# XiangFeng-Wen/STF-Unet

Measured on AMD Instinct MI355X. Metric: training samples/sec (256x256 DCE-MRI frames), higher is better.
Workload: dtype bf16; 1 GPU; cfg2 UNet(in=8,base_c=64) 256x256 train step; model=UNet, global_batch=64, per_gpu_batch=64, seq_len=8, parallelism=dp1, ddp_hook=False

## Files before the change

### include/stfunet.h

```cpp
#ifndef STFUNET_H
#define STFUNET_H
#include <stddef.h>
#include <stdint.h>

#ifdef __cplusplus
extern "C" {
#endif

typedef void* stf_stream_t;

typedef struct stf_conv_geom {
  int N;
  int Hs, Ws, Cs;
  int src_cstride;
  int Hd, Wd;
  int R, S;
  int stride, pad;
  int transposed;
} stf_conv_geom;

typedef struct stf_lstm_epi {
  const float* c_prev;
  float* c_out;
  void* h_out;
// ... 66 lines not shown
                    float* scale, float* shift, stf_stream_t stream);
typedef struct stf_bn_run_desc {
  const float* stats;
  float* running_mean;
  float* running_var;
  int64_t Mg;
  int tiles, groups, C;
  float momentum;
} stf_bn_run_desc;
int stf_bn_running_batch(const stf_bn_run_desc* descs, int count, stf_stream_t stream);
int stf_bn_act(const void* y, int y_cstride, int N, int H, int W, int C, int groups,
               const float* scale, const float* shift, int relu, const void* res,
               int res_cstride, const float* res_scale, const float* res_shift, void* out,
               int out_cstride, void* pooled, stf_stream_t stream);
int stf_bn_bwd_tiles(int N, int H, int W, int C, int groups, int pooled);
int stf_bn_bwd_reduce(const void* dz, int dz_cstride, const void* dpool, const void* y,
                      int y_cstride, int N, int H, int W, int C, int groups,
                      const float* scale, const float* shift, const float* mean,
                      const float* invstd, int mask_mode, const void* mask_src,
                      int mask_cstride, void* g_out, float* partial, stf_stream_t stream);
int stf_bn_bwd_finalize(float* partial, int tiles, int groups, int C, int64_t M,
                        const float* gamma, const float* mean, const float* invstd,
                        float* dgamma, float* dbeta, float* coef, stf_stream_t stream);
typedef struct stf_bn_gsum_desc {
  const float* partial;
  float* dgamma;
  float* dbeta;
  int tiles, groups, C;
} stf_bn_gsum_desc;
int stf_bn_groupsum_batch(const stf_bn_gsum_desc* descs, int count, stf_stream_t stream);
int stf_bn_bwd_apply_tiles(int64_t M, int C);
int stf_bn_bwd_apply(const void* g, int g_cstride, const void* y, int y_cstride, int64_t M,
                     int C, int groups, const float* mask_scale, const float* mask_shift,
                     const float* coef, void* dy, int dy_cstride, float* bias_partial,
                     float* dbias, stf_stream_t stream);

int stf_head_fwd(const void* y, int N, int H, int W, int C, const float* scale,
                 const float* shift, const float* w, const float* bias, int classes,
                 float* logits, stf_stream_t stream);
int stf_head_bwd(const float* dlogits, const void* y, int N, int H, int W, int C,
                 const float* scale, const float* shift, const float* mean,
                 const float* invstd, const float* w, int classes, void* g_out,
                 float* bn_partial, float* head_partial, float* dw, float* db,
                 stf_stream_t stream);
int stf_head_tiles(int N, int H, int W, int C);

// ... 276 lines not shown
```

### stf-unet_amd/csrc/bn.hip

```cpp
#include <algorithm>

#include "common.h"
#include "../../include/stfunet.h"
#include "reduce.h"

namespace {

constexpr int NT = 256;

STF_DEV void bn_fin_store(int g, int c, int C, double mu, double var, const float* gamma, const float* beta,
                          float eps, float* mean, float* invstd, float* scale, float* shift) {
  const float inv = (float)(1.0 / sqrt(var + (double)eps));
  const float sc = gamma[c] * inv;
  mean[g * C + c] = (float)mu;
  invstd[g * C + c] = inv;
  scale[g * C + c] = sc;
  shift[g * C + c] = beta[c] - (float)mu * sc;
}

STF_DEV void bn_fin_fwd_out(float* base, int g, int c, int G, int C, long Mg, double s1, double s2,
                            const float* gamma, const float* beta, float mom, float eps, float* rm, float* rv,
                            float* mean, float* invstd, float* scale, float* shift) {
  const double mu = s1 / Mg;
  double var = s2 / Mg - mu * mu;
// ... 29 lines not shown
  if (!lead) return;
  bn_fin_store(g, c, C, rm ? rm[c] : 0.f, rv ? rv[c] : 1.f, gamma, beta, eps, mean, invstd, scale, shift);
}

STF_DEV void bn_fin_bwd_out(float* base, int g, int c, int G, int C, long Mg, double s1, double s2,
                            const float* gamma, const float* mean, const float* invstd, float* dgamma, float* dbeta,
                            float* coef) {
  const double is = invstd[g * C + c];
  const double A = (double)gamma[c] * is;
  const double B = -A * is * s2 / Mg;
  const double Cc = -A * s1 / Mg + A * is * mean[g * C + c] * s2 / Mg;
  coef[(size_t)g * 3 * C + c] = (float)A;
  coef[(size_t)g * 3 * C + C + c] = (float)B;
  coef[(size_t)g * 3 * C + 2 * C + c] = (float)Cc;
  if (G == 1) {
    if (dgamma) dgamma[c] = (float)s2;
    if (dbeta) dbeta[c] = (float)s1;
  } else {
    base[c] = (float)s1;
    base[C + c] = (float)s2;
  }
}


STF_DEV void load_pair(const float* a, const float* b, int g, int C, int cg, float (&va)[8], float (&vb)[8]) {
  load8f(a + (size_t)g * C, cg * 8, va);
  load8f(b + (size_t)g * C, cg * 8, vb);
}
STF_DEV void load_coef(const float* coef, int g, int C, int cg, float (&A)[8], float (&B)[8], float (&Cc)[8]) {
  load8f(coef + (size_t)g * 3 * C, cg * 8, A);
  load8f(coef + (size_t)g * 3 * C + C, cg * 8, B);
  load8f(coef + (size_t)g * 3 * C + 2 * C, cg * 8, Cc);
}

STF_DEV void bn_affine8(float (&v)[8], const float (&sc)[8], const float (&sh)[8], int relu, int res_mode,
                        const uint4* rq, const float (&rs)[8], const float (&rh)[8]) {
#pragma unroll
  for (int j = 0; j < 8; ++j) v[j] = v[j] * sc[j] + sh[j];
  if (res_mode) {
    float r[8];
    unpack8(*rq, r);
    if (res_mode == 2) {
#pragma unroll
      for (int j = 0; j < 8; ++j) r[j] = r[j] * rs[j] + rh[j];
    }
#pragma unroll
// ... 11 lines not shown
  for (int j = 0; j < 8; ++j) {
    bool keep = true;
    if (mask == 1) keep = y[j] * sc[j] + sh[j] > 0.f;
    else if (mask == 2) keep = mk[j] > 0.f;
    const float gj = keep ? d[j] : 0.f;
    d[j] = gj;
    sg[j] += gj;
    sgx[j] += gj * (y[j] - mu[j]) * is[j];
  }
}

STF_DEV void bn_dy8(bool mask, float (&gv)[8], const float (&y)[8], const float (&ms)[8], const float (&mh)[8],
                    const float (&A)[8], const float (&B)[8], const float (&Cc)[8], float (&sb)[8]) {
#pragma unroll
  for (int j = 0; j < 8; ++j) {
    const float gj = (mask && !(y[j] * ms[j] + mh[j] > 0.f)) ? 0.f : gv[j];
    gv[j] = A[j] * gj + B[j] * y[j] + Cc[j];
    sb[j] += gv[j];
  }
}

template <int Q = 1, int NTH, int RW>
STF_DEV void bn_block_fold(float (&red)[NTH][RW], const float (&s0)[8], const float (&s1)[8], int C, int stride,
                           int gy, float* __restrict__ out) {
  constexpr int H = (RW - 1) / 8;
#pragma unroll
  for (int j = 0; j < 8; ++j) {
    red[threadIdx.x][j] = s0[j];
    if (H == 2) red[threadIdx.x][8 + j] = s1[j];
  }
  __syncthreads();
  const size_t row = (size_t)gy * gridDim.x + blockIdx.x;
  for (int c = threadIdx.x; c < C; c += NTH) {
    const int gg = c >> 3, j = c & 7;
    float a = 0.f, b = 0.f;
    for (int t = Q * gg; t < NTH; t += stride)
      for (int q = 0; q < Q; ++q) {
        a += red[t + q][j];
        if (H == 2) b += red[t + q][8 + j];
      }
    out[row * H * C + c] = a;
    if (H == 2) out[row * H * C + C + c] = b;
  }
}

template <bool POOL>
__global__ void bn_act_kernel(const uint16_t* __restrict__ y, int ycs, long N, int H, int W, int C, long Mg,
                              const float* scale, const float* shift, int relu, int res_mode,
                              const uint16_t* __restrict__ res, int rcs, const float* __restrict__ rscale,
                              const float* __restrict__ rshift, uint16_t* __restrict__ out, int ocs,
                              uint16_t* __restrict__ pooled) {
  const int CG = C / 8;
  const long units = POOL ? N * (H / 2) * (W / 2) * CG : N * H * W * CG;
  for (long u = blockIdx.x * (long)NT + threadIdx.x; u < units; u += (long)gridDim.x * NT) {
    const int cg = (int)(u % CG);
    const long pix = u / CG;
    if (!POOL) {
      const int g = (int)(pix / Mg);
      float sc[8], sh[8], v[8];
      load_pair(scale, shift, g, C, cg, sc, sh);
      unpack8(*reinterpret_cast<const uint4*>(y + pix * ycs + cg * 8), v);
#pragma unroll
      for (int j = 0; j < 8; ++j) v[j] = v[j] * sc[j] + sh[j];
      if (res_mode) {
        float r[8];
// ... 102 lines not shown
        sg[j] += t;
        sgx[j] += t * (v[d][j] - mu[j]) * is[j];
      }
      *reinterpret_cast<uint4*>(g_out + p[d] * C + cg * 8) = pack8(gd);
    }
  }
  bn_block_fold(red, sg, sgx, C, CG, 0, partial);
}

STF_DEV float quad_xor1(float v) {
  return __int_as_float(__builtin_amdgcn_mov_dpp(__float_as_int(v), 0xB1, 0xF, 0xF, false));
}
STF_DEV float quad_xor2(float v) {
  return __int_as_float(__builtin_amdgcn_mov_dpp(__float_as_int(v), 0x4E, 0xF, 0xF, false));
}

constexpr int PNT = 512;
__global__ __launch_bounds__(PNT) void bn_bwd_reduce_pool_kernel(const uint16_t* __restrict__ dz, int dzcs,
                                          const uint16_t* __restrict__ dpool, const uint16_t* __restrict__ y,
                                          int ycs, long N, int H, int W, int C, int G, int tpg,
                                          const float* __restrict__ scale, const float* __restrict__ shift,
                                          const float* __restrict__ mean, const float* __restrict__ invstd,
                                          int mask_mode, uint16_t* __restrict__ g_out,
                                          float* __restrict__ partial) {
  __shared__ float red[PNT][17];
  const int CG = C / 8;
  const int g = blockIdx.x / tpg, tile = blockIdx.x - g * tpg;
  const int Wp = W / 2, Hp = H / 2;
  const long wpg = (N / G) * Hp * Wp;
  const long U = wpg * CG * 4;
  const long gt = (long)tile * PNT + threadIdx.x;
  const int d = (int)(gt & 3);
  const int cg = (int)((gt >> 2) % CG);
  float sc[8], sh[8], mu[8], is[8];
  load_pair(scale, shift, g, C, cg, sc, sh);
  load_pair(mean, invstd, g, C, cg, mu, is);
  const bool relu = mask_mode == 1;
  float sg[8] = {0, 0, 0, 0, 0, 0, 0, 0}, sgx[8] = {0, 0, 0, 0, 0, 0, 0, 0};
  const int HpWp = Hp * Wp, cshift = __builtin_ctz(CG);
  const long S = (long)tpg * PNT;
  auto pix = [&](long u, int& win) {
    win = (int)(u >> (2 + cshift)) + (int)(g * wpg);
    const int n = win / HpWp;
    const int rem = win - n * HpWp;
    const int py = rem / Wp, px = rem - py * Wp;
    return ((long)(n * H + 2 * py + (d >> 1))) * W + 2 * px + (d & 1);
  };
  auto unit = [&](long p, int win, const uint4& yv, const uint4& zv, const uint4& pv) {
// ... 20 lines not shown
      sg[j] += gj;
      sgx[j] += gj * (v[j] - mu[j]) * is[j];
    }
    *reinterpret_cast<uint4*>(g_out + p * C + cg * 8) = pack8(gd);
  };
  const uint4 zero4 = make_uint4(0, 0, 0, 0);
  for (long u = gt; u < U; u += 2 * S) {
    const bool two = u + S < U;
    int w0, w1 = 0;
    const long p0 = pix(u, w0);
    const long p1 = two ? pix(u + S, w1) : p0;
    const uint4 y0 = *reinterpret_cast<const uint4*>(y + p0 * ycs + cg * 8);
    const uint4 z0 = dz ? *reinterpret_cast<const uint4*>(dz + p0 * dzcs + cg * 8) : zero4;
    const uint4 q0 = *reinterpret_cast<const uint4*>(dpool + (long)w0 * C + cg * 8);
    uint4 y1 = zero4, z1 = zero4, q1 = zero4;
    if (two) {
      y1 = *reinterpret_cast<const uint4*>(y + p1 * ycs + cg * 8);
      if (dz) z1 = *reinterpret_cast<const uint4*>(dz + p1 * dzcs + cg * 8);
      q1 = *reinterpret_cast<const uint4*>(dpool + (long)w1 * C + cg * 8);
    }
    unit(p0, w0, y0, z0, q0);
    if (two) unit(p1, w1, y1, z1, q1);
  }
  bn_block_fold<4>(red, sg, sgx, C, 4 * CG, 0, partial);
}

__global__ __launch_bounds__(stf::FOLD_NT) void bn_bwd_finalize_kernel(float* __restrict__ partial, int S, int T, int G,
                                                            int C, long Mg, const float* gamma, const float* mean,
                                                            const float* invstd, float* dgamma, float* dbeta,
                                                            float* coef) {
  __shared__ double red[stf::FOLD_NT];
  const int g = blockIdx.y;
  const int c = blockIdx.x * 16 + (threadIdx.x & 15);
  const bool cok = c < C, lead = cok && (threadIdx.x >> 4) == 0;
  float* base = partial + (size_t)g * T * 2 * C;
  double s1, s2;
  stf::fold16_pair(base, S, 2L * C, C, c, cok, red, s1, s2);
  if (lead) bn_fin_bwd_out(base, g, c, G, C, Mg, s1, s2, gamma, mean, invstd, dgamma, dbeta, coef);
}

constexpr int RUN_BATCH = 32;
struct RunBatch { stf_bn_run_desc d[RUN_BATCH]; };
__global__ void bn_running_batch_kernel(RunBatch b) {
  const stf_bn_run_desc& d = b.d[blockIdx.y];
  const int c = blockIdx.x * blockDim.x + threadIdx.x;
  if (c >= d.C) return;
  float run_m = d.running_mean[c], run_v = d.running_var[c];
// ... 52 lines not shown
        if (RES) rv[k] = *reinterpret_cast<const uint4*>(res + p * rcs + cg * 8);
      }
    }
#pragma unroll
    for (int k = 0; k < UPT; ++k) {
      const int uk = u + k * NT;
      if (uk >= upg) break;
      float v[8];
      unpack8(yv[k], v);
      bn_affine8(v, sc, sh, relu, RES ? (res_mode == 2 ? 2 : 1) : 0, &rv[k], rs, rh);
      *reinterpret_cast<uint4*>(out + (p0 + (uk >> cgs)) * ocs + cg * 8) = pack8(v);
    }
  }
}

template <int MASK>
__global__ __launch_bounds__(NT) void bn_bwd_reduce_g_kernel(const uint16_t* __restrict__ dz, int dzcs,
                                                             const uint16_t* __restrict__ y, int ycs, int Mg,
                                                             int cgs, const float* __restrict__ scale,
                                                             const float* __restrict__ shift,
                                                             const float* __restrict__ mean,
                                                             const float* __restrict__ invstd,
                                                             const uint16_t* __restrict__ msrc, int mcs,
                                                             uint16_t* __restrict__ g_out, float* __restrict__ partial) {
  __shared__ float red[NT][17];
  const int g = blockIdx.y, CG = 1 << cgs, C = 8 << cgs;
  const int upg = Mg << cgs, S = gridDim.x * NT * UPT;
  const int u0 = blockIdx.x * NT * UPT + threadIdx.x;
  const int cg = threadIdx.x & (CG - 1);
  float sc[8], sh[8], mu[8], is[8];
  if (MASK == 1) load_pair(scale, shift, g, C, cg, sc, sh);
  load_pair(mean, invstd, g, C, cg, mu, is);
  float sg[8] = {0, 0, 0, 0, 0, 0, 0, 0}, sgx[8] = {0, 0, 0, 0, 0, 0, 0, 0};
  const size_t p0 = (size_t)g * Mg;
  for (int u = u0; u < upg; u += S) {
    uint4 yv[UPT], zv[UPT], mv[UPT];
#pragma unroll
    for (int k = 0; k < UPT; ++k) {
      const int uk = u + k * NT;
      if (uk < upg) {
        const size_t p = p0 + (uk >> cgs);
        yv[k] = *reinterpret_cast<const uint4*>(y + p * ycs + cg * 8);
        zv[k] = *reinterpret_cast<const uint4*>(dz + p * dzcs + cg * 8);
        if (MASK == 2) mv[k] = *reinterpret_cast<const uint4*>(msrc + p * mcs + cg * 8);
      }
    }
#pragma unroll
    for (int k = 0; k < UPT; ++k) {
      const int uk = u + k * NT;
      if (uk >= upg) break;
      float v[8], d[8], mk[8];
      unpack8(yv[k], v);
      unpack8(zv[k], d);
      if (MASK == 2) unpack8(mv[k], mk);
      bn_acc8(MASK, d, v, sc, sh, mk, mu, is, sg, sgx);
      if (g_out) *reinterpret_cast<uint4*>(g_out + (p0 + (uk >> cgs)) * C + cg * 8) = pack8(d);
    }
  }
  bn_block_fold(red, sg, sgx, C, CG, g, partial);
}

template <bool MASK>
__global__ __launch_bounds__(NT) void bn_bwd_apply_g_kernel(const uint16_t* g_in, int gcs,
                                                            const uint16_t* __restrict__ y, int ycs, int Mg, int cgs,
                                                            const float* coef, const float* __restrict__ mscale,
                                                            const float* __restrict__ mshift, uint16_t* dy,
                                                            int dycs, float* __restrict__ bias_partial) {
  __shared__ float red[NT][9];
  const int g = blockIdx.y, CG = 1 << cgs, C = 8 << cgs;
  const int upg = Mg << cgs, S = gridDim.x * NT * UPT;
  const int u0 = blockIdx.x * NT * UPT + threadIdx.x;
  const int cg = threadIdx.x & (CG - 1);
  float A[8], B[8], Cc[8], ms[8], mh[8];
  load_coef(coef, g, C, cg, A, B, Cc);
  if (MASK) load_pair(mscale, mshift, g, C, cg, ms, mh);
  float sb[8] = {0, 0, 0, 0, 0, 0, 0, 0};
  const size_t p0 = (size_t)g * Mg;
  for (int u = u0; u < upg; u += S) {
    uint4 gq[UPT], yq[UPT];
#pragma unroll
    for (int k = 0; k < UPT; ++k) {
      const int uk = u + k * NT;
// ... 161 lines not shown
enum class BnOp { Act, Reduce, Apply, ActPool3, ReducePool3, ApplyPool3 };
struct BnSig {
  BnOp op;
  long N;
  int H, W, C, groups;
  bool pooled = false;
  int mask = 0;
  bool res = false;
  bool bias = false;
};
enum class BnKernel {
  None, ActG, ActGRes, ActFlat, ActFlatPool, ReduceG0, ReduceG1, ReduceG2, ReduceDpp, ReduceWin, ApplyG, ApplyGMask,
  ActPool3, ReducePool3, ApplyPool3
};
struct BnRoute {
  bool refused = true;
  BnKernel kernel = BnKernel::None;
  int block = NT;
  dim3 grid;
  int rows = 0;
  int alloc = 1;
  int cgs = 0;
  long Mg = 0;
};

constexpr long ROW_CAP = stf::FOLD16_ROWS, BLOCK_CAP = 8192, IDX_CAP = 1L << 31;

BnRoute bn_route(const BnSig& s) {
  BnRoute r;
  if (s.groups < 1) return r;
  const auto clamp = [](long want, long most) { return (int)std::max<long>(1, std::min(want, most)); };
  const auto ceil_div = [](long x, long y) { return (x + y - 1) / y; };
  const int CG = s.C / 8, Ho = (s.H - 1) / 2 + 1, Wo = (s.W - 1) / 2 + 1;
  const long Ng = s.N / s.groups, px = s.N * s.H * s.W;
  r.Mg = Ng * s.H * s.W;
  const bool chunk_ok = s.C >= 8 && s.C % 8 == 0 && NT % CG == 0;
  const bool g_ok = chunk_ok && r.Mg * CG < IDX_CAP;
  if (chunk_ok) r.cgs = 31 - __builtin_clz(CG);
  const bool uneven = s.N % s.groups != 0, odd = ((s.H | s.W) & 1) != 0;
  const long upg = Ng * CG * (s.op == BnOp::ApplyPool3 ? (long)((s.H + 1) / 2) * ((s.W + 1) / 2)
                              : s.pooled ? (long)(s.H / 2) * (s.W / 2) : (long)s.H * s.W);
  const auto rows_of = [&](long units) { return clamp(ceil_div(units, NT), ceil_div(ROW_CAP, s.groups)); };
  const auto blocks_of = [&](long cap) { return clamp(ceil_div(upg, (long)NT * UPT), cap / s.groups); };
  const auto flat = [&](long units) { return (unsigned)std::min(ceil_div(units, NT), BLOCK_CAP); };
  switch (s.op) {
    case BnOp::Act:
      r.refused = s.C % 8 || uneven || (s.pooled && (odd || s.res));
      if (!s.pooled && g_ok) {
        r.kernel = s.res ? BnKernel::ActGRes : BnKernel::ActG;
        r.grid = dim3(upg ? blocks_of(BLOCK_CAP) : 0, s.groups);
      } else {
        r.kernel = s.pooled ? BnKernel::ActFlatPool : BnKernel::ActFlat;
        r.grid = dim3(flat(upg * s.groups));
      }
      break;
    case BnOp::Reduce:
      r.refused = !chunk_ok || uneven || (s.pooled ? odd || s.mask == 2 : !g_ok);
      r.rows = r.alloc = rows_of(upg);
      if (!s.pooled) {
        r.kernel = s.mask == 1 ? BnKernel::ReduceG1 : s.mask == 2 ? BnKernel::ReduceG2 : BnKernel::ReduceG0;
        r.grid = dim3(r.rows, s.groups);
      } else {
        const bool dpp = chunk_ok && 64 % CG == 0 && px < IDX_CAP;
        r.kernel = dpp ? BnKernel::ReduceDpp : BnKernel::ReduceWin;
        r.block = dpp ? PNT : NT;
        r.grid = dim3(r.rows * s.groups);
      }
      break;
    case BnOp::Apply:
      r.alloc = clamp(ceil_div(px * CG, NT), ROW_CAP);
      r.rows = blocks_of(s.bias ? r.alloc : BLOCK_CAP);
      r.refused = !g_ok || uneven || (s.bias && (long)r.rows * s.groups > r.alloc);
      r.kernel = s.mask ? BnKernel::ApplyGMask : BnKernel::ApplyG;
      r.grid = dim3(r.rows, s.groups);
      if (!s.bias) r.rows = 0;
      break;
    case BnOp::ActPool3: {
      const long units = s.N * Ho * Wo * CG;
      r.refused = s.C % 8 || uneven || units >= IDX_CAP - BLOCK_CAP * NT || px * s.C >= IDX_CAP * 8;
      r.kernel = BnKernel::ActPool3;
      r.grid = dim3(std::max(flat(units), 1u));
      break;
    }
    case BnOp::ReducePool3:
      r.refused = !g_ok || uneven || px >= IDX_CAP;
      r.kernel = BnKernel::ReducePool3;
      r.rows = r.alloc = rows_of(r.Mg * CG);
      r.grid = dim3(r.rows, s.groups);
      break;
    case BnOp::ApplyPool3:
// ... 49 lines not shown
                       r.cgs, scale, shift, relu, res_mode, (const uint16_t*)res, res_cstride, res_scale, res_shift,
                       (uint16_t*)out, out_cstride);
  };
  const auto flat = [&](auto kernel) {
    hipLaunchKernelGGL(kernel, r.grid, dim3(r.block), 0, (hipStream_t)stream, (const uint16_t*)y, y_cstride, (long)N, H,
                       W, C, r.Mg, scale, shift, relu, res_mode, (const uint16_t*)res, res_cstride, res_scale,
                       res_shift, (uint16_t*)out, out_cstride, (uint16_t*)pooled);
  };
  switch (r.kernel) {
    case BnKernel::ActG: group_major(bn_act_g_kernel<false>); break;
    case BnKernel::ActGRes: group_major(bn_act_g_kernel<true>); break;
    case BnKernel::ActFlat: flat(bn_act_kernel<false>); break;
    case BnKernel::ActFlatPool: flat(bn_act_kernel<true>); break;
    default: return STF_EINVAL;
  }
  STF_CHECK_LAUNCH();
  return 0;
}

extern "C" int stf_bn_bwd_tiles(int N, int H, int W, int C, int groups, int pooled) {
  return bn_route({BnOp::Reduce, N, H, W, C, groups, pooled != 0}).alloc;
}

extern "C" int stf_bn_bwd_reduce(const void* dz, int dz_cstride, const void* dpool, const void* y, int y_cstride,
                                 int N, int H, int W, int C, int groups, const float* scale, const float* shift,
                                 const float* mean, const float* invstd, int mask_mode, const void* mask_src,
                                 int mask_cstride, void* g_out, float* partial, stf_stream_t stream) {
  const BnRoute r = bn_route({BnOp::Reduce, N, H, W, C, groups, dpool != nullptr, mask_mode});
  if (r.refused || y_cstride % 8 || (dz && dz_cstride % 8)) return STF_EINVAL;
  if (!dz && !dpool) return STF_EINVAL;
  if (!g_out && dpool) return STF_EINVAL;
  if (mask_mode == 2 && (!mask_src || mask_cstride % 8)) return STF_EINVAL;
  hipStream_t s = (hipStream_t)stream;
  const auto group_major = [&](auto kernel) {
    hipLaunchKernelGGL(kernel, r.grid, dim3(r.block), 0, s, (const uint16_t*)dz, dz_cstride, (const uint16_t*)y,
                       y_cstride, (int)r.Mg, r.cgs, scale, shift, mean, invstd, (const uint16_t*)mask_src,
                       mask_cstride, (uint16_t*)g_out, partial);
  };
  switch (r.kernel) {
    case BnKernel::ReduceG0: group_major(bn_bwd_reduce_g_kernel<0>); break;
    case BnKernel::ReduceG1: group_major(bn_bwd_reduce_g_kernel<1>); break;
    case BnKernel::ReduceG2: group_major(bn_bwd_reduce_g_kernel<2>); break;
    case BnKernel::ReduceDpp:
      hipLaunchKernelGGL(bn_bwd_reduce_pool_kernel, r.grid, dim3(r.block), 0, s, (const uint16_t*)dz, dz_cstride,
                         (const uint16_t*)dpool, (const uint16_t*)y, y_cstride, (long)N, H, W, C, groups, r.rows, scale,
                         shift, mean, invstd, mask_mode, (uint16_t*)g_out, partial);
      break;
    case BnKernel::ReduceWin:
      hipLaunchKernelGGL(bn_bwd_reduce_win_kernel, r.grid, dim3(r.block), 0, s, (const uint16_t*)dz, dz_cstride,
                         (const uint16_t*)dpool, (const uint16_t*)y, y_cstride, (long)N, H, W, C, groups, r.rows, scale,
                         shift, mean, invstd, mask_mode, (const uint16_t*)mask_src, mask_cstride, (uint16_t*)g_out,
                         partial);
      break;
    default: return STF_EINVAL;
  }
  STF_CHECK_LAUNCH();
  return 0;
}

extern "C" int stf_bn_bwd_finalize(float* partial, int tiles, int groups, int C, int64_t M, const float* gamma,
                                   const float* mean, const float* invstd, float* dgamma, float* dbeta, float* coef,
                                   stf_stream_t stream) {
  hipStream_t s = (hipStream_t)stream;
  if (groups < 1 || M % groups) return STF_EINVAL;
  const int S = stf::colsum_stage1(partial, tiles, 2L * C, s, groups, stf::FOLD16_ROWS);
  hipLaunchKernelGGL(bn_bwd_finalize_kernel, dim3((C + 15) / 16, groups), dim3(stf::FOLD_NT), 0, s, partial, S, tiles, groups,
                     C, (long)(M / groups), gamma, mean, invstd, dgamma, dbeta, coef);
  STF_CHECK_LAUNCH();
  if (groups > 1 && (dgamma || dbeta)) {
    GsumBatch b;
    b.d[0] = stf_bn_gsum_desc{partial, dgamma, dbeta, tiles, groups, C};
    hipLaunchKernelGGL(bn_groupsum_batch_kernel, dim3((C + 255) / 256, 1), dim3(256), 0, s, b);
    STF_CHECK_LAUNCH();
  }
  return 0;
}

extern "C" int stf_bn_running_batch(const stf_bn_run_desc* descs, int count, stf_stream_t stream) {
  for (int i = 0; i < count; ++i)
    if (!descs[i].stats || !descs[i].running_mean || !descs[i].running_var || descs[i].groups < 1 ||
// ... 96 lines not shown
```

### stf-unet_amd/csrc/reduce.h

```cpp
#pragma once
#include "common.h"

namespace stf {

static __global__ void colsum_inplace_kernel(float* __restrict__ buf, long T, long W, int S) {
  const long j = blockIdx.x * (long)blockDim.x + threadIdx.x;
  const int s = blockIdx.y;
  if (j >= W) return;
  float* b = buf + (size_t)blockIdx.z * T * W;
  double acc = 0.0;
  for (long t = s; t < T; t += S) acc += b[t * W + j];
  b[(long)s * W + j] = (float)acc;
}

static inline int colsum_split(long T, long W, int G) {
  long s = T / 64;
  const long blocks_x = (W + 255) / 256;
  if (blocks_x * s * G < 512) s = T / 16;
  if (s < 1) s = 1;
  if (s > 256) s = 256;
  if (s > T) s = (int)T;
  return (int)s;
}

// ... 12 lines not shown
    int t = threadIdx.x >> 4;
    for (; t + 3 * RL < S; t += 4 * RL) {
      a0 += base[(long)t * stride + c];
      a1 += base[(long)(t + RL) * stride + c];
      a2 += base[(long)(t + 2 * RL) * stride + c];
      a3 += base[(long)(t + 3 * RL) * stride + c];
    }
    for (; t < S; t += RL) a0 += base[(long)t * stride + c];
  }
  return (a0 + a1) + (a2 + a3);
}

STF_DEV double fold16_finish(double v, double* red) {
  red[threadIdx.x] = v;
  __syncthreads();
  double tot = 0.0;
  const int RL = blockDim.x >> 4;
  if ((threadIdx.x >> 4) == 0)
    for (int r = 0; r < RL; ++r) tot += red[r * 16 + (threadIdx.x & 15)];
  __syncthreads();
  return tot;
}

STF_DEV void fold16_pair(const float* base, int S, long stride, long off2, long c, bool cok, double* red,
                         double& o1, double& o2) {
  double a0 = 0.0, a1 = 0.0, b0 = 0.0, b1 = 0.0;
  if (cok) {
    const int RL = blockDim.x >> 4;
    int t = threadIdx.x >> 4;
    for (; t + RL < S; t += 2 * RL) {
      const float x0 = base[(long)t * stride + c], y0 = base[(long)t * stride + off2 + c];
      const float x1 = base[(long)(t + RL) * stride + c], y1 = base[(long)(t + RL) * stride + off2 + c];
      a0 += x0; b0 += y0; a1 += x1; b1 += y1;
    }
    for (; t < S; t += RL) {
      a0 += base[(long)t * stride + c];
      b0 += base[(long)t * stride + off2 + c];
    }
  }
  double v1 = a0 + a1, v2 = b0 + b1;
  v1 += __shfl_xor(v1, 16, 64);
  v2 += __shfl_xor(v2, 16, 64);
  v1 += __shfl_xor(v1, 32, 64);
  v2 += __shfl_xor(v2, 32, 64);
  const int wave = threadIdx.x >> 6, nw = blockDim.x >> 6, lane = threadIdx.x & 63;
  if (lane < 16) {
    red[wave * 16 + lane] = v1;
    red[(nw + wave) * 16 + lane] = v2;
  }
  __syncthreads();
  o1 = o2 = 0.0;
  if (threadIdx.x < 16)
    for (int w = 0; w < nw; ++w) {
      o1 += red[w * 16 + threadIdx.x];
      o2 += red[(nw + w) * 16 + threadIdx.x];
    }
}

constexpr int FOLD_NT = 1024;

constexpr long FOLD16_ROWS = 1024;

}
```

### stf-unet_amd/stfunet/_lib.py

```python
import contextlib
import ctypes
import os

import torch

_HERE = os.path.dirname(os.path.abspath(__file__))
LIB_PATH = os.path.join(_HERE, "libstfunet_hip.so")
LIB_PATH = os.environ.get("STF_LIB", LIB_PATH)
LIB_PATH_F16 = os.environ.get("STF_LIB_F16", os.path.join(os.path.dirname(LIB_PATH), "libstfunet_hip_f16.so"))
LIB_PATHS = {torch.bfloat16: LIB_PATH, torch.float16: LIB_PATH_F16}
STORAGE_CODE = {torch.bfloat16: 0, torch.float16: 1}

BUILD_INFO = os.path.join(_HERE, "build_info.json")
_SRC_DIRS = (os.path.join(_HERE, "..", "csrc"), os.path.join(_HERE, "..", "..", "include"))


def _sha(paths):
    import hashlib
    h = hashlib.sha256()
    for p in paths:
        h.update(os.path.basename(p).encode())
        with open(p, "rb") as f:
            h.update(f.read())
    return h.hexdigest()[:16]
# ... 68 lines not shown
    _fields_ = [("model", P), ("off", c_int64), ("len", c_int64)]


_SIGS = {
    "stf_igemm_stat_tiles": (c_int, [ctypes.POINTER(IgemmArgs)]),
    "stf_igemm_ws_bytes": (c_size_t, [ctypes.POINTER(IgemmArgs)]),
    "stf_igemm_bnr_tiles": (c_int, [ctypes.POINTER(IgemmArgs)]),
    "stf_igemm_kernel_name": (ctypes.c_char_p, [ctypes.POINTER(IgemmArgs)]),
    "stf_wgrad_kernel_name": (ctypes.c_char_p, [ctypes.POINTER(WgradArgs)]),
    "stf_igemm": (c_int, [ctypes.POINTER(IgemmArgs), P]),
    "stf_wgrad_plan": (c_int, [ctypes.POINTER(WgradArgs), ctypes.POINTER(c_int), ctypes.POINTER(c_size_t)]),
    "stf_wgrad": (c_int, [ctypes.POINTER(WgradArgs), P]),
    "stf_wgrad_reduce": (c_int, [P, c_int, c_int, c_int, c_int, c_int, P, P]),
    "stf_channel_sum": (c_int, [P, c_int, c_int, c_int, P, P, P]),
    "stf_bn_finalize": (c_int, [P, c_int, c_int, c_int, c_int64, P, P, c_float, c_float, P, P, P, P, P, P, P]),
    "stf_bn_running_batch": (c_int, [P, c_int, P]),
    "stf_bn_groupsum_batch": (c_int, [P, c_int, P]),
    "stf_bn_act": (c_int, [P, c_int, c_int, c_int, c_int, c_int, c_int, P, P, c_int, P, c_int, P, P, P, c_int, P,
                           P]),
    "stf_bn_bwd_tiles": (c_int, [c_int, c_int, c_int, c_int, c_int, c_int]),
    "stf_bn_bwd_reduce": (c_int, [P, c_int, P, P, c_int, c_int, c_int, c_int, c_int, c_int, P, P, P, P, c_int, P,
                                  c_int, P, P, P]),
    "stf_bn_bwd_finalize": (c_int, [P, c_int, c_int, c_int, c_int64, P, P, P, P, P, P, P]),
    "stf_bn_bwd_apply_tiles": (c_int, [c_int64, c_int]),
    "stf_bn_bwd_apply": (c_int, [P, c_int, P, c_int, c_int64, c_int, c_int, P, P, P, P, c_int, P, P, P]),
    "stf_head_fwd": (c_int, [P, c_int, c_int, c_int, c_int, P, P, P, P, c_int, P, P]),
    "stf_head_bwd": (c_int, [P, P, c_int, c_int, c_int, c_int, P, P, P, P, P, c_int, P, P, P, P, P, P]),
    "stf_head_tiles": (c_int, [c_int, c_int, c_int, c_int]),
    "stf_loss_scratch_floats": (c_int, [c_int, c_int]),
    "stf_loss_fwd": (c_int, [P, P, c_int, c_int, c_int, c_int, P, P, P]),
    "stf_loss_bwd": (c_int, [P, P, c_int, c_int, c_int, c_int, P, P, P, P]),
    "stf_loss_opt_scratch_floats": (c_int, [c_int, c_int]),
    "stf_loss_opt_fwd": (c_int, [P, P, c_int, c_int, c_int, c_int, P, c_int, c_int, P, P, P]),
    "stf_loss_opt_bwd": (c_int, [P, P, c_int, c_int, c_int, c_int, P, c_int, c_int, P, P, P, P]),
    "stf_head_mc_fwd": (c_int, [P, c_int, c_int, c_int, c_int, P, P, P, P, c_int, P, P]),
    "stf_head_mc_bwd": (c_int, [P, P, c_int, c_int, c_int, c_int, P, P, P, P, P, c_int, P, P, P, P, P, P]),
    "stf_loss_mc_scratch_floats": (c_int, [c_int, c_int]),
    "stf_loss_mc_fwd": (c_int, [P, P, c_int, c_int, c_int, c_int, P, c_int, c_int, P, P, P]),
    "stf_loss_mc_bwd": (c_int, [P, P, c_int, c_int, c_int, c_int, P, c_int, c_int, P, P, P, P]),
    "stf_loss_ft_scratch_floats": (c_int, [c_int, c_int]),
    "stf_loss_ft_fwd": (c_int, [P, P, c_int, c_int, c_int, c_int, P, c_int, c_int, c_float, c_float, c_float, P, P,
                                P]),
    "stf_loss_ft_bwd": (c_int, [P, P, c_int, c_int, c_int, c_int, P, c_int, c_int, c_float, c_float, c_float, P, P,
                                P, P]),
    "stf_adamw": (c_int, [P, P, P, P, c_int64, c_float, c_float, c_float, c_float, c_float, c_float, c_float,
                          P]),
# ... 195 lines not shown
```

### stf-unet_amd/stfunet/nhwc.py

```python
import contextlib
import ctypes
import os
from dataclasses import dataclass

import torch

from . import _lib
from ._lib import BnrEpi, ConvGeom, IgemmArgs, WgradArgs, call, stream

BF16 = torch.bfloat16


def sdt():
    return _lib.storage_dtype()


def _p(t):
    return t.data_ptr() if t is not None else None


class KernelTimer:

    def __init__(self, only=None, log=False):
        self.rec = {}
# ... 555 lines not shown
         _p(res_st.scale) if res_st is not None else None, _p(res_st.shift) if res_st is not None else None,
         out.ptr(), out.cs, pooled.ptr() if pooled is not None else None, stream())


def bn_backward(y: Feat, st: BNState, bn, dgamma, dbeta, dz: Feat = None, dpool: Feat = None, relu=True,
                dbias=None, mask: Feat = None, out: Feat = None, keep_g=False):
    y.check()
    C = y.C
    dev = y.buf.device
    G = st.groups
    tiles = _lib.load().stf_bn_bwd_tiles(y.N, y.H, y.W, C, G, int(dpool is not None))
    part = empty(G * tiles * 2 * C, torch.float32, dev)
    if dz is not None:
        dz.check()
        assert (dz.N, dz.H, dz.W, dz.C) == (y.N, y.H, y.W, C)
    if dpool is not None:
        dpool.check()
        assert dpool.cs == C and dpool.off == 0 and (dpool.H, dpool.W) == (y.H // 2, y.W // 2)
    mode = 2 if mask is not None else (1 if relu else 0)
    if mask is not None:
        mask.check()
    direct = dpool is None and mode != 2 and not keep_g
    g = None if direct else new_feat(y.N, y.H, y.W, C, dev)
    call("stf_bn_bwd_reduce", dz.ptr() if dz is not None else None, dz.cs if dz is not None else 0,
         dpool.ptr() if dpool is not None else None, y.ptr(), y.cs, y.N, y.H, y.W, C, G, _p(st.scale),
         _p(st.shift), _p(st.mean), _p(st.invstd), mode, mask.ptr() if mask is not None else None,
         mask.cs if mask is not None else 0, g.ptr() if g is not None else None, _p(part), stream())
    if keep_g and out is None:
        out = new_feat(y.N, y.H, y.W, C, dev)
    if direct:
        if out is None:
            out = new_feat(y.N, y.H, y.W, C, dev)
        dy = bn_backward_from_partial(dz, y, st, bn, part, tiles, dgamma, dbeta, dbias, out=out,
                                      mask_relu=(mode == 1))
    else:
        dy = bn_backward_from_partial(g, y, st, bn, part, tiles, dgamma, dbeta, dbias, out=out)
    return (dy, g) if keep_g else dy


def bn_backward_fused(dz: Feat, y: Feat, st: BNState, bn, part, tiles, dgamma, dbeta, dbias=None, relu=True):
    assert dz.cs == dz.C and dz.off == 0
    return bn_backward_from_partial(dz, y, st, bn, part, tiles, dgamma, dbeta, dbias, out=dz if relu else None,
                                    mask_relu=relu)


def bn_backward_maxpool3(y: Feat, st: BNState, bn, dgamma, dbeta, argmax, dpool: Feat):
    y.check()
    dpool.check()
    C, dev, G = y.C, y.buf.device, st.groups
    assert y.cs == C and y.off == 0 and dpool.cs == C and dpool.off == 0
    assert (dpool.N, dpool.H, dpool.W) == (y.N, (y.H - 1) // 2 + 1, (y.W - 1) // 2 + 1)
    tiles = _lib.load().stf_bn_bwd_tiles(y.N, y.H, y.W, C, G, 0)
    part = empty(G * tiles * 2 * C, torch.float32, dev)
    call("stf_bn_bwd_reduce_pool3", _p(argmax), dpool.ptr(), y.ptr(), y.N, y.H, y.W, C, G, _p(st.scale),
         _p(st.shift), _p(st.mean), _p(st.invstd), _p(part), stream())
    coef = _bn_bwd_coef(y, st, bn, part, tiles, dgamma, dbeta)
    dy = new_feat(y.N, y.H, y.W, C, dev)
    call("stf_bn_bwd_apply_pool3", _p(argmax), dpool.ptr(), y.ptr(), y.N, y.H, y.W, C, G, _p(st.scale),
         _p(st.shift), _p(coef), dy.ptr(), stream())
    return dy


def _bn_bwd_coef(y: Feat, st: BNState, bn, part, tiles, dgamma, dbeta):
    C, dev, G = y.C, y.buf.device, st.groups
    coef = empty(G * 3 * C, torch.float32, dev)
    if G > 1 and (dgamma is not None or dbeta is not None):
        _GSUM_PENDING.append((_GsumDesc(part.data_ptr(), dgamma.data_ptr() if dgamma is not None else None,
                                        dbeta.data_ptr() if dbeta is not None else None, tiles, G, C), part))
        dgamma = dbeta = None
    call("stf_bn_bwd_finalize", _p(part), tiles, G, C, y.M, bn.weight.data_ptr(), _p(st.mean),
         _p(st.invstd), _p(dgamma), _p(dbeta), _p(coef), stream())
    if not st.training:
        cv = coef.view(G, 3, C)
        cv[:, 0].copy_(bn.weight.detach() * st.invstd)
        cv[:, 1:].zero_()
    return coef


def bn_backward_from_partial(g: Feat, y: Feat, st: BNState, bn, part, tiles, dgamma, dbeta, dbias=None,
                             out: Feat = None, mask_relu=False):
    C = y.C
    dev = y.buf.device
    G = st.groups
    if st.training:
        dbias = None
    coef = _bn_bwd_coef(y, st, bn, part, tiles, dgamma, dbeta)
    bpart = None
    if dbias is not None:
        bpart = empty(_lib.load().stf_bn_bwd_apply_tiles(y.M, C) * C, torch.float32, dev)
    dst = out if out is not None else g
    if out is not None:
        out.check()
        assert (out.N, out.H, out.W, out.C) == (y.N, y.H, y.W, C)
    if mask_relu:
        assert out is not None
    call("stf_bn_bwd_apply", g.ptr(), g.cs, y.ptr(), y.cs, y.M, C, G, _p(st.scale) if mask_relu else None,
         _p(st.shift) if mask_relu else None, _p(coef), dst.ptr(), dst.cs, _p(bpart), _p(dbias), stream())
    return dst


MAX_CLASSES = 16


def check_num_classes(K):
    if not 1 <= K <= MAX_CLASSES:
        raise ValueError(f"num_classes={K}: the head and criterion kernels take 1 to {MAX_CLASSES} classes")


def _head_entry(name, K):
# ... 26 lines not shown
```

Before: 2728 samples/s.

## Fuse BN backward finalize into reduce kernel via last-block atomic fold

BN backward reduce kernels now publish their per-block partials with agent-scope atomic stores and count arrivals on a per-stream device counter. The last block to arrive folds all partials and writes dgamma, dbeta and the backward coefficients, so the separate finalize launch is skipped for single-group training layers with enough blocks. This removes one kernel launch and its dependency gap per BN layer in backward. In exchange it adds a global atomic, a fence, and a serial tail fold inside one block, which needs correct memory ordering.

```diff
diff --git a/include/stfunet.h b/include/stfunet.h
--- a/include/stfunet.h
+++ b/include/stfunet.h
@@ -112,6 +112,13 @@
 int stf_bn_bwd_finalize(float* partial, int tiles, int groups, int C, int64_t M,
                         const float* gamma, const float* mean, const float* invstd,
                         float* dgamma, float* dbeta, float* coef, stf_stream_t stream);
+int stf_bn_bwd_fold(int N, int H, int W, int C, int groups, int pooled, int training);
+int stf_bn_bwd_reduce_fin(const void* dz, int dz_cstride, const void* dpool, const void* y,
+                          int y_cstride, int N, int H, int W, int C, const float* scale,
+                          const float* shift, const float* mean, const float* invstd,
+                          int mask_mode, const void* mask_src, int mask_cstride, void* g_out,
+                          float* partial, const float* gamma, float* dgamma, float* dbeta,
+                          float* coef, stf_stream_t stream);
 typedef struct stf_bn_gsum_desc {
   const float* partial;
   float* dgamma;
diff --git a/stf-unet_amd/csrc/bn.hip b/stf-unet_amd/csrc/bn.hip
--- a/stf-unet_amd/csrc/bn.hip
+++ b/stf-unet_amd/csrc/bn.hip
@@ -75,6 +75,29 @@
   }
 }
 
+struct BwdFin {
+  const float* gamma;
+  float *dgamma, *dbeta, *coef;
+  unsigned* counter;
+  long Mg;
+};
+
+template <int NTH>
+STF_DEV void bn_bwd_fin_last(float* lds, float* partial, int rows, int C, const BwdFin& f, const float* mean,
+                             const float* invstd) {
+  static_assert(2 * (stf::FOLD_NT / 64) * 16 * sizeof(double) < (NTH * 17 - 1) * sizeof(float), "fold scratch");
+  if (!stf::arrive_last(f.counter, gridDim.x * gridDim.y, reinterpret_cast<unsigned*>(lds) + NTH * 17 - 1)) return;
+  double* red = reinterpret_cast<double*>(lds);
+  for (int c0 = 0; c0 < C; c0 += 16) {
+    const int c = c0 + (threadIdx.x & 15);
+    const bool cok = c < C;
+    double s1, s2;
+    stf::fold16_pair_as<NTH>(partial, rows, 2L * C, C, c, cok, red, s1, s2);
+    if (cok && threadIdx.x < 16)
+      bn_fin_bwd_out(partial, 0, c, 1, C, f.Mg, s1, s2, f.gamma, mean, invstd, f.dgamma, f.dbeta, f.coef);
+  }
+}
+
 
 STF_DEV void load_pair(const float* a, const float* b, int g, int C, int cg, float (&va)[8], float (&vb)[8]) {
   load8f(a + (size_t)g * C, cg * 8, va);
@@ -132,7 +155,7 @@
 
 template <int Q = 1, int NTH, int RW>
 STF_DEV void bn_block_fold(float (&red)[NTH][RW], const float (&s0)[8], const float (&s1)[8], int C, int stride,
-                           int gy, float* __restrict__ out) {
+                           int gy, float* __restrict__ out, bool through = false) {
   constexpr int H = (RW - 1) / 8;
 #pragma unroll
   for (int j = 0; j < 8; ++j) {
@@ -149,8 +172,13 @@
         a += red[t + q][j];
         if (H == 2) b += red[t + q][8 + j];
       }
-    out[row * H * C + c] = a;
-    if (H == 2) out[row * H * C + C + c] = b;
+    if (through) {
+      __hip_atomic_store(out + row * H * C + c, a, __ATOMIC_RELAXED, __HIP_MEMORY_SCOPE_AGENT);
+      if (H == 2) __hip_atomic_store(out + row * H * C + C + c, b, __ATOMIC_RELAXED, __HIP_MEMORY_SCOPE_AGENT);
+    } else {
+      out[row * H * C + c] = a;
+      if (H == 2) out[row * H * C + C + c] = b;
+    }
   }
 }
 
@@ -299,8 +327,8 @@
                                           const float* __restrict__ scale, const float* __restrict__ shift,
                                           const float* __restrict__ mean, const float* __restrict__ invstd,
                                           int mask_mode, uint16_t* __restrict__ g_out,
-                                          float* __restrict__ partial) {
-  __shared__ float red[PNT][17];
+                                          float* __restrict__ partial, BwdFin fin) {
+  __shared__ __attribute__((aligned(16))) float red[PNT][17];
   const int CG = C / 8;
   const int g = blockIdx.x / tpg, tile = blockIdx.x - g * tpg;
   const int Wp = W / 2, Hp = H / 2;
@@ -367,7 +395,8 @@
     unit(p0, w0, y0, z0, q0);
     if (two) unit(p1, w1, y1, z1, q1);
   }
-  bn_block_fold<4>(red, sg, sgx, C, 4 * CG, 0, partial);
+  bn_block_fold<4>(red, sg, sgx, C, 4 * CG, 0, partial, fin.coef != nullptr);
+  if (fin.coef) bn_bwd_fin_last<PNT>(&red[0][0], partial, gridDim.x, C, fin, mean, invstd);
 }
 
 __global__ __launch_bounds__(stf::FOLD_NT) void bn_bwd_finalize_kernel(float* __restrict__ partial, int S, int T, int G,
@@ -466,8 +495,9 @@
                                                              const float* __restrict__ mean,
                                                              const float* __restrict__ invstd,
                                                              const uint16_t* __restrict__ msrc, int mcs,
-                                                             uint16_t* __restrict__ g_out, float* __restrict__ partial) {
-  __shared__ float red[NT][17];
+                                                             uint16_t* __restrict__ g_out, float* __restrict__ partial,
+                                                             BwdFin fin) {
+  __shared__ __attribute__((aligned(16))) float red[NT][17];
   const int g = blockIdx.y, CG = 1 << cgs, C = 8 << cgs;
   const int upg = Mg << cgs, S = gridDim.x * NT * UPT;
   const int u0 = blockIdx.x * NT * UPT + threadIdx.x;
@@ -501,7 +531,8 @@
       if (g_out) *reinterpret_cast<uint4*>(g_out + (p0 + (uk >> cgs)) * C + cg * 8) = pack8(d);
     }
   }
-  bn_block_fold(red, sg, sgx, C, CG, g, partial);
+  bn_block_fold(red, sg, sgx, C, CG, g, partial, fin.coef != nullptr);
+  if (fin.coef) bn_bwd_fin_last<NT>(&red[0][0], partial, gridDim.x, C, fin, mean, invstd);
 }
 
 template <bool MASK>
@@ -709,9 +740,11 @@
   int alloc = 1;
   int cgs = 0;
   long Mg = 0;
+  bool fin_ok = false;
+  bool fold = false;
 };
 
-constexpr long ROW_CAP = stf::FOLD16_ROWS, BLOCK_CAP = 8192, IDX_CAP = 1L << 31;
+constexpr long ROW_CAP = stf::FOLD16_ROWS, BLOCK_CAP = 8192, IDX_CAP = 1L << 31, FOLD_MIN_BLOCKS = 256;
 
 BnRoute bn_route(const BnSig& s) {
   BnRoute r;
@@ -753,6 +786,8 @@
         r.block = dpp ? PNT : NT;
         r.grid = dim3(r.rows * s.groups);
       }
+      r.fin_ok = !r.refused && s.groups == 1 && r.kernel != BnKernel::ReduceWin;
+      r.fold = r.fin_ok && r.rows >= FOLD_MIN_BLOCKS;
       break;
     case BnOp::Apply:
       r.alloc = clamp(ceil_div(px * CG, NT), ROW_CAP);
@@ -848,20 +883,28 @@
   return bn_route({BnOp::Reduce, N, H, W, C, groups, pooled != 0}).alloc;
 }
 
-extern "C" int stf_bn_bwd_reduce(const void* dz, int dz_cstride, const void* dpool, const void* y, int y_cstride,
-                                 int N, int H, int W, int C, int groups, const float* scale, const float* shift,
-                                 const float* mean, const float* invstd, int mask_mode, const void* mask_src,
-                                 int mask_cstride, void* g_out, float* partial, stf_stream_t stream) {
+extern "C" int stf_bn_bwd_fold(int N, int H, int W, int C, int groups, int pooled, int training) {
+  return training && bn_route({BnOp::Reduce, N, H, W, C, groups, pooled != 0}).fold;
+}
+
+static int bn_bwd_reduce(const void* dz, int dz_cstride, const void* dpool, const void* y, int y_cstride, int N,
+                         int H, int W, int C, int groups, const float* scale, const float* shift, const float* mean,
+                         const float* invstd, int mask_mode, const void* mask_src, int mask_cstride, void* g_out,
+                         float* partial, const float* gamma, float* dgamma, float* dbeta, float* coef,
+                         stf_stream_t stream) {
   const BnRoute r = bn_route({BnOp::Reduce, N, H, W, C, groups, dpool != nullptr, mask_mode});
   if (r.refused || y_cstride % 8 || (dz && dz_cstride % 8)) return STF_EINVAL;
   if (!dz && !dpool) return STF_EINVAL;
   if (!g_out && dpool) return STF_EINVAL;
   if (mask_mode == 2 && (!mask_src || mask_cstride % 8)) return STF_EINVAL;
+  if (coef && (groups != 1 || !gamma)) return STF_EINVAL;
   hipStream_t s = (hipStream_t)stream;
+  BwdFin fin{gamma, dgamma, dbeta, nullptr, nullptr, r.Mg};
+  if (coef && r.fin_ok && (fin.counter = stf::fold_counter(s)) != nullptr) fin.coef = coef;
   const auto group_major = [&](auto kernel) {
     hipLaunchKernelGGL(kernel, r.grid, dim3(r.block), 0, s, (const uint16_t*)dz, dz_cstride, (const uint16_t*)y,
                        y_cstride, (int)r.Mg, r.cgs, scale, shift, mean, invstd, (const uint16_t*)mask_src,
-                       mask_cstride, (uint16_t*)g_out, partial);
+                       mask_cstride, (uint16_t*)g_out, partial, fin);
   };
   switch (r.kernel) {
     case BnKernel::ReduceG0: group_major(bn_bwd_reduce_g_kernel<0>); break;
@@ -870,7 +913,7 @@
     case BnKernel::ReduceDpp:
       hipLaunchKernelGGL(bn_bwd_reduce_pool_kernel, r.grid, dim3(r.block), 0, s, (const uint16_t*)dz, dz_cstride,
                          (const uint16_t*)dpool, (const uint16_t*)y, y_cstride, (long)N, H, W, C, groups, r.rows, scale,
-                         shift, mean, invstd, mask_mode, (uint16_t*)g_out, partial);
+                         shift, mean, invstd, mask_mode, (uint16_t*)g_out, partial, fin);
       break;
     case BnKernel::ReduceWin:
       hipLaunchKernelGGL(bn_bwd_reduce_win_kernel, r.grid, dim3(r.block), 0, s, (const uint16_t*)dz, dz_cstride,
@@ -881,7 +924,27 @@
     default: return STF_EINVAL;
   }
   STF_CHECK_LAUNCH();
+  if (coef && !fin.coef)
+    return stf_bn_bwd_finalize(partial, r.rows, 1, C, (int64_t)r.Mg, gamma, mean, invstd, dgamma, dbeta, coef, stream);
   return 0;
+}
+
+extern "C" int stf_bn_bwd_reduce(const void* dz, int dz_cstride, const void* dpool, const void* y, int y_cstride,
+                                 int N, int H, int W, int C, int groups, const float* scale, const float* shift,
+                                 const float* mean, const float* invstd, int mask_mode, const void* mask_src,
+                                 int mask_cstride, void* g_out, float* partial, stf_stream_t stream) {
+  return bn_bwd_reduce(dz, dz_cstride, dpool, y, y_cstride, N, H, W, C, groups, scale, shift, mean, invstd, mask_mode,
+                       mask_src, mask_cstride, g_out, partial, nullptr, nullptr, nullptr, nullptr, stream);
+}
+
+extern "C" int stf_bn_bwd_reduce_fin(const void* dz, int dz_cstride, const void* dpool, const void* y, int y_cstride,
+                                     int N, int H, int W, int C, const float* scale, const float* shift,
+                                     const float* mean, const float* invstd, int mask_mode, const void* mask_src,
+                                     int mask_cstride, void* g_out, float* partial, const float* gamma,
+                                     float* dgamma, float* dbeta, float* coef, stf_stream_t stream) {
+  if (!coef) return STF_EINVAL;
+  return bn_bwd_reduce(dz, dz_cstride, dpool, y, y_cstride, N, H, W, C, 1, scale, shift, mean, invstd, mask_mode,
+                       mask_src, mask_cstride, g_out, partial, gamma, dgamma, dbeta, coef, stream);
 }
 
 extern "C" int stf_bn_bwd_finalize(float* partial, int tiles, int groups, int C, int64_t M, const float* gamma,
diff --git a/stf-unet_amd/csrc/reduce.h b/stf-unet_amd/csrc/reduce.h
--- a/stf-unet_amd/csrc/reduce.h
+++ b/stf-unet_amd/csrc/reduce.h
@@ -1,4 +1,6 @@
 #pragma once
+#include <mutex>
+
 #include "common.h"
 
 namespace stf {
@@ -58,12 +60,12 @@
   return tot;
 }
 
-STF_DEV void fold16_pair(const float* base, int S, long stride, long off2, long c, bool cok, double* red,
-                         double& o1, double& o2) {
+STF_DEV void fold16_pair_lane(const float* base, int S, long stride, long off2, long c, bool cok, double* red,
+                              int vt, int nt) {
   double a0 = 0.0, a1 = 0.0, b0 = 0.0, b1 = 0.0;
   if (cok) {
-    const int RL = blockDim.x >> 4;
-    int t = threadIdx.x >> 4;
+    const int RL = nt >> 4;
+    int t = vt >> 4;
     for (; t + RL < S; t += 2 * RL) {
       const float x0 = base[(long)t * stride + c], y0 = base[(long)t * stride + off2 + c];
       const float x1 = base[(long)(t + RL) * stride + c], y1 = base[(long)(t + RL) * stride + off2 + c];
@@ -79,12 +81,15 @@
   v2 += __shfl_xor(v2, 16, 64);
   v1 += __shfl_xor(v1, 32, 64);
   v2 += __shfl_xor(v2, 32, 64);
-  const int wave = threadIdx.x >> 6, nw = blockDim.x >> 6, lane = threadIdx.x & 63;
+  const int wave = vt >> 6, nw = nt >> 6, lane = vt & 63;
   if (lane < 16) {
     red[wave * 16 + lane] = v1;
     red[(nw + wave) * 16 + lane] = v2;
   }
-  __syncthreads();
+}
+
+STF_DEV void fold16_pair_sum(const double* red, int nt, double& o1, double& o2) {
+  const int nw = nt >> 6;
   o1 = o2 = 0.0;
   if (threadIdx.x < 16)
     for (int w = 0; w < nw; ++w) {
@@ -93,8 +98,67 @@
     }
 }
 
+STF_DEV void fold16_pair(const float* base, int S, long stride, long off2, long c, bool cok, double* red,
+                         double& o1, double& o2) {
+  fold16_pair_lane(base, S, stride, off2, c, cok, red, threadIdx.x, blockDim.x);
+  __syncthreads();
+  fold16_pair_sum(red, blockDim.x, o1, o2);
+}
+
 constexpr int FOLD_NT = 1024;
 
 constexpr long FOLD16_ROWS = 1024;
 
+template <int NTH>
+STF_DEV void fold16_pair_as(const float* base, int S, long stride, long off2, long c, bool cok, double* red,
+                            double& o1, double& o2) {
+  static_assert(NTH % 64 == 0 && FOLD_NT % NTH == 0, "whole waves, whole passes");
+  for (int vt = threadIdx.x; vt < FOLD_NT; vt += NTH) fold16_pair_lane(base, S, stride, off2, c, cok, red, vt, FOLD_NT);
+  __syncthreads();
+  fold16_pair_sum(red, FOLD_NT, o1, o2);
+  __syncthreads();
 }
+
+STF_DEV bool arrive_last(unsigned* counter, unsigned count, unsigned* flag) {
+  asm volatile("s_waitcnt vmcnt(0)" ::: "memory");
+  __syncthreads();
+  if (threadIdx.x == 0) {
+    const unsigned ticket = __hip_atomic_fetch_add(counter, 1u, __ATOMIC_RELAXED, __HIP_MEMORY_SCOPE_AGENT);
+    const bool last = ticket + 1 == count;
+    if (last) {
+      __hip_atomic_store(counter, 0u, __ATOMIC_RELAXED, __HIP_MEMORY_SCOPE_AGENT);
+      __builtin_amdgcn_fence(__ATOMIC_ACQUIRE, "agent");
+      asm volatile("s_waitcnt vmcnt(0)" ::: "memory");
+    }
+    *flag = last;
+  }
+  __syncthreads();
+  const bool last = *flag != 0;
+  __syncthreads();
+  return last;
+}
+
+constexpr int FOLD_SLOTS = 64;
+static __device__ unsigned fold_counters[FOLD_SLOTS];
+
+static inline unsigned* fold_counter(hipStream_t s) {
+  struct Key { int dev; hipStream_t s; };
+  static std::mutex mu;
+  static Key keys[FOLD_SLOTS];
+  static unsigned* base[FOLD_SLOTS];
+  static int used = 0;
+  int dev = 0;
+  if (hipGetDevice(&dev) != hipSuccess) return nullptr;
+  std::lock_guard<std::mutex> lock(mu);
+  for (int i = 0; i < used; ++i)
+    if (keys[i].dev == dev && keys[i].s == s) return base[i] + i;
+  if (used == FOLD_SLOTS) return nullptr;
+  void* p = nullptr;
+  if (hipGetSymbolAddress(&p, HIP_SYMBOL(fold_counters)) != hipSuccess || !p) return nullptr;
+  const int i = used++;
+  keys[i] = Key{dev, s};
+  base[i] = (unsigned*)p;
+  return base[i] + i;
+}
+
+}
diff --git a/stf-unet_amd/stfunet/_lib.py b/stf-unet_amd/stfunet/_lib.py
--- a/stf-unet_amd/stfunet/_lib.py
+++ b/stf-unet_amd/stfunet/_lib.py
@@ -114,6 +114,9 @@
     "stf_bn_bwd_reduce": (c_int, [P, c_int, P, P, c_int, c_int, c_int, c_int, c_int, c_int, P, P, P, P, c_int, P,
                                   c_int, P, P, P]),
     "stf_bn_bwd_finalize": (c_int, [P, c_int, c_int, c_int, c_int64, P, P, P, P, P, P, P]),
+    "stf_bn_bwd_fold": (c_int, [c_int, c_int, c_int, c_int, c_int, c_int, c_int]),
+    "stf_bn_bwd_reduce_fin": (c_int, [P, c_int, P, P, c_int, c_int, c_int, c_int, c_int, P, P, P, P, c_int, P,
+                                      c_int, P, P, P, P, P, P, P]),
     "stf_bn_bwd_apply_tiles": (c_int, [c_int64, c_int]),
     "stf_bn_bwd_apply": (c_int, [P, c_int, P, c_int, c_int64, c_int, c_int, P, P, P, P, c_int, P, P, P]),
     "stf_head_fwd": (c_int, [P, c_int, c_int, c_int, c_int, P, P, P, P, c_int, P, P]),
diff --git a/stf-unet_amd/stfunet/nhwc.py b/stf-unet_amd/stfunet/nhwc.py
--- a/stf-unet_amd/stfunet/nhwc.py
+++ b/stf-unet_amd/stfunet/nhwc.py
@@ -601,20 +601,37 @@
         mask.check()
     direct = dpool is None and mode != 2 and not keep_g
     g = None if direct else new_feat(y.N, y.H, y.W, C, dev)
-    call("stf_bn_bwd_reduce", dz.ptr() if dz is not None else None, dz.cs if dz is not None else 0,
-         dpool.ptr() if dpool is not None else None, y.ptr(), y.cs, y.N, y.H, y.W, C, G, _p(st.scale),
-         _p(st.shift), _p(st.mean), _p(st.invstd), mode, mask.ptr() if mask is not None else None,
-         mask.cs if mask is not None else 0, g.ptr() if g is not None else None, _p(part), stream())
+    head = (dz.ptr() if dz is not None else None, dz.cs if dz is not None else 0,
+            dpool.ptr() if dpool is not None else None, y.ptr(), y.cs, y.N, y.H, y.W, C)
+    tail = (_p(st.scale), _p(st.shift), _p(st.mean), _p(st.invstd), mode, mask.ptr() if mask is not None else None,
+            mask.cs if mask is not None else 0, g.ptr() if g is not None else None, _p(part))
+    coef = None
+    if _bn_bwd_fold(y, G, dpool is not None, st.training):
+        coef = empty(3 * C, torch.float32, dev)
+        call("stf_bn_bwd_reduce_fin", *head, *tail, bn.weight.data_ptr(), _p(dgamma), _p(dbeta), _p(coef), stream())
+    else:
+        call("stf_bn_bwd_reduce", *head, G, *tail, stream())
     if keep_g and out is None:
         out = new_feat(y.N, y.H, y.W, C, dev)
     if direct:
         if out is None:
             out = new_feat(y.N, y.H, y.W, C, dev)
         dy = bn_backward_from_partial(dz, y, st, bn, part, tiles, dgamma, dbeta, dbias, out=out,
-                                      mask_relu=(mode == 1))
+                                      mask_relu=(mode == 1), coef=coef)
     else:
-        dy = bn_backward_from_partial(g, y, st, bn, part, tiles, dgamma, dbeta, dbias, out=out)
+        dy = bn_backward_from_partial(g, y, st, bn, part, tiles, dgamma, dbeta, dbias, out=out, coef=coef)
     return (dy, g) if keep_g else dy
+
+
+_BN_FOLD = {}
+
+
+def _bn_bwd_fold(y: Feat, G, pooled, training):
+    key = (y.N, y.H, y.W, y.C, G, pooled, training)
+    f = _BN_FOLD.get(key)
+    if f is None:
+        f = _BN_FOLD[key] = bool(_lib.load().stf_bn_bwd_fold(y.N, y.H, y.W, y.C, G, int(pooled), int(training)))
+    return f
 
 
 def bn_backward_fused(dz: Feat, y: Feat, st: BNState, bn, part, tiles, dgamma, dbeta, dbias=None, relu=True):
@@ -657,13 +674,14 @@
 
 
 def bn_backward_from_partial(g: Feat, y: Feat, st: BNState, bn, part, tiles, dgamma, dbeta, dbias=None,
-                             out: Feat = None, mask_relu=False):
+                             out: Feat = None, mask_relu=False, coef=None):
     C = y.C
     dev = y.buf.device
     G = st.groups
     if st.training:
         dbias = None
-    coef = _bn_bwd_coef(y, st, bn, part, tiles, dgamma, dbeta)
+    if coef is None:
+        coef = _bn_bwd_coef(y, st, bn, part, tiles, dgamma, dbeta)
     bpart = None
     if dbias is not None:
         bpart = empty(_lib.load().stf_bn_bwd_apply_tiles(y.M, C) * C, torch.float32, dev)
```

Result: slower. 2578 samples/s (-5.5%).
